# Henningson/Fireflies

Measured on AMD Instinct MI355X. Metric: renders/sec @512x512,64spp vocal-fold (+ pattern-grad-steps/sec in grad_steps_per_sec); HBM GB/s vs peak in roofline, higher is better.
Workload: dtype f32

## Files before the change

fireflies_amd/csrc/ffx_trace.hip:

```cpp
#include <stdlib.h>
#include <string.h>

#include <limits.h>

#include "ffx_common.h"
#include "ffx_band.h"
#include "../../include/ffx_labels.h"

#define TR_BLOCK 256
#define RAY_EPS 8.940696716308594e-05f
#define SHADOW_EPS (10.0f * RAY_EPS)

struct CamK {
  float s2c[16];
  float tw[12];
  float near_clip, far_clip, inv_w, inv_h;
  int W, H;
  int w_uniform;
  float iw_u;
};

struct RfC { float alpha, bias, aL, aL2, k[4]; int rec; };
enum { FFX_PRE_ETA, FFX_PRE_INV_ETA2, FFX_PRE_A2, FFX_PRE_INV_A2, FFX_PRE_METALLIC, FFX_PRE_C_SW, FFX_PRE_C_FD, FFX_PRE_BRDF, FFX_PRE_ROUGH2, FFX_PRE_FLAGS, FFX_PRE_R2,
       FFX_PRE_TINT_TERM, FFX_PRE_FLOATS  };
#define FFX_PRE_ANISO 1u
#define FFX_PRE_TINT 2u
#define FFX_PRE_CLEARCOAT 4u
#define FFX_PRE_FLAT 8u
#define FFX_PRE_SHEEN 16u
// ... 9 lines not shown
  float s_pos[3], s_int[3];
  float cos_cut, cos_beam, cutoff, inv_trans;
  int s_rigid;
  int mat_stride;
  const float *mats;
  int n_base_tex;
  int btw[FFX_MAX_BASE_TEX], bth[FFX_MAX_BASE_TEX];
  const float *btex[FFX_MAX_BASE_TEX];
  const float *slot_uv;
  int mat_inline;
  float mat_h[FFX_MAX_MAT_H];
  int mat_pre_on;
  float mat_pre[8 * FFX_PRE_FLOATS];
  BinsK bins;
  RfC rf;
};
template <typename T>
__device__ __forceinline__ const T &kernarg_first() {
  const __attribute__((address_space(4))) char *p = (const __attribute__((address_space(4))) char *)__builtin_amdgcn_kernarg_segment_ptr();
  asm volatile("" : "+s"(p));
  return *(const T *)p;
}
__device__ __forceinline__ const ShadeK &kernarg_shade() { return kernarg_first<ShadeK>(); }
__device__ __forceinline__ const float *mat_table(const ShadeK &k) { return k.mat_inline ? k.mat_h : k.mats; }

struct Hit { float t; int prim, shape, slot; };

struct RayBox { v3 o, id; };
#define FFX_TIE_WIDEN 1.0000004f
__device__ __forceinline__ float safe_rcp_dir(float d) {
  float a = fabsf(d) < 1e-20f ? copysignf(1e-20f, d) : d;
  return __builtin_amdgcn_rcpf(a);
}
__device__ __forceinline__ RayBox make_raybox(v3 o, v3 d) {
  RayBox r;
  r.o = o;
  r.id = V3(safe_rcp_dir(d.x), safe_rcp_dir(d.y), safe_rcp_dir(d.z));
  return r;
}
__device__ __forceinline__ bool slab(const float lo[3], const float hi[3], const RayBox &rb, float tmin, float tmax, float &tn_out) {
  float ax = (lo[0] - rb.o.x) * rb.id.x, bx = (hi[0] - rb.o.x) * rb.id.x;
  float ay = (lo[1] - rb.o.y) * rb.id.y, by = (hi[1] - rb.o.y) * rb.id.y;
  float az = (lo[2] - rb.o.z) * rb.id.z, bz = (hi[2] - rb.o.z) * rb.id.z;
  float tn = fmaxf(fmaxf(fminf(ax, bx), fminf(ay, by)), fmaxf(fminf(az, bz), tmin));
  float tf = fminf(fminf(fmaxf(ax, bx), fmaxf(ay, by)), fmaxf(az, bz)) * 1.0000004f;
  tf = fminf(tf, tmax);
// ... 103 lines not shown
      if (sp == 0) break;
      --sp;
      cur = stack[sp * stride];
    }
  }
  return h.prim >= 0;
}

__device__ __forceinline__ void sample_jitter(uint32_t seed_key, uint32_t idx, float &jx, float &jy) {
  uint32_t a = hash32((2u * idx) ^ seed_key), b = hash32((2u * idx + 1u) ^ seed_key);
  jx = (float)(a >> 8) * (1.0f / 16777216.0f);
  jy = (float)(b >> 8) * (1.0f / 16777216.0f);
}

#ifdef FFX_K8_NO_BAND
#define FFX_K8_BAND false
#else
#define FFX_K8_BAND true
#endif
#ifdef FFX_K8_NO_OFF32
#define FFX_K8_OFF32 false
#else
#define FFX_K8_OFF32 true
#endif
template <bool BAND = false>
__device__ __forceinline__ void cam_ray(const CamK &k, float sx, float sy, v3 &o, v3 &d, float &near_t, float &far_t) {
  const float *m = k.s2c;
  float qx = fmaf(m[0], sx, fmaf(m[1], sy, m[3]));
  float qy = fmaf(m[4], sx, fmaf(m[5], sy, m[7]));
  float qz = fmaf(m[8], sx, fmaf(m[9], sy, m[11]));
  float iw;
  if (BAND || k.w_uniform) iw = k.iw_u;
  else iw = 1.0f / fmaf(m[12], sx, fmaf(m[13], sy, m[15]));
  v3 np = V3(qx * iw, qy * iw, qz * iw);
  const float il = BAND ? rcp_band(sqrt_band(vdot(np, np))) : 1.0f / sqrtf(vdot(np, np));
  v3 dl = V3(np.x * il, np.y * il, np.z * il);
  d = xf_dir(k.tw, dl);
  o = V3(k.tw[3], k.tw[7], k.tw[11]);
  const float idz = BAND ? rcp_band(dl.z) : 1.0f / dl.z;
  near_t = k.near_clip * idz;
  far_t = k.far_clip * idz;
}

__global__ void __launch_bounds__(TR_BLOCK)
    k_trace_primary(CamK cam, const BvhNode *__restrict__ nodes, const TriRec *__restrict__ recs, int spp, int jitter, uint32_t seed_key, long total,
                    float *__restrict__ t_out, int32_t *__restrict__ shape_out, int32_t *__restrict__ prim_out) {
// ... 1388 lines not shown
    return;
  }
  const float scale = 0.999f * __builtin_amdgcn_rcpf(tmax);
  const RayOct rb = make_rayoct(o, d, scale);
  const uint32_t oct = (__float_as_uint(rb.id.x) >> 31) | ((__float_as_uint(rb.id.y) >> 31) << 1) | ((__float_as_uint(rb.id.z) >> 31) << 2);
  const uint32_t oct0 = (uint32_t)__builtin_amdgcn_readlane((int)oct, __builtin_ctzll(am));
  const bool uniform = (am & __builtin_amdgcn_uicmp(oct, oct0, 33)) == 0ull;
  if (uniform) {
    switch (oct0) {
      case 0: traverse_packet_oct<ANY, 0>(nodes, arecs, rb, scale, d, tmin, tmax, am, h, found); break;
      case 1: traverse_packet_oct<ANY, 1>(nodes, arecs, rb, scale, d, tmin, tmax, am, h, found); break;
      case 2: traverse_packet_oct<ANY, 2>(nodes, arecs, rb, scale, d, tmin, tmax, am, h, found); break;
      case 3: traverse_packet_oct<ANY, 3>(nodes, arecs, rb, scale, d, tmin, tmax, am, h, found); break;
      case 4: traverse_packet_oct<ANY, 4>(nodes, arecs, rb, scale, d, tmin, tmax, am, h, found); break;
      case 5: traverse_packet_oct<ANY, 5>(nodes, arecs, rb, scale, d, tmin, tmax, am, h, found); break;
      case 6: traverse_packet_oct<ANY, 6>(nodes, arecs, rb, scale, d, tmin, tmax, am, h, found); break;
      default: traverse_packet_oct<ANY, 7>(nodes, arecs, rb, scale, d, tmin, tmax, am, h, found); break;
    }
  } else {
    traverse_packet<ANY>(nodes, arecs, o, d, tmin, tmax, active, h, found);
  }
}

template <bool ANY, bool OFF32 = false>
__device__ __forceinline__ void traverse_bins(const char *__restrict__ bbase, const int nx, const int tx0, const int ty0, const int tx1, const int ty1, const float rcx,
                                              const float rcy, const float rhx, const float rhy, const TriApex *__restrict__ recs, const v3 d, const float tmin,
                                              const float tmax, const wmask active, Hit &h, wmask &occluded) {
  h.t = msel(active, tmax, -INFINITY);
  h.prim = -1;
  h.shape = -1;
  h.slot = -1;
  occluded = 0ull;
  const uint32_t lane = threadIdx.x & 63u;
  const uint32_t *starts = reinterpret_cast<const uint32_t *>(bbase + 64);
  const char *ents = bbase + ffx_bin_off_entries();
  const char *rbase = reinterpret_cast<const char *>(recs);
  auto uni = [](float v) { return __int_as_float(__builtin_amdgcn_readfirstlane(__float_as_int(v))); };
  const float rx0 = uni(rcx - rhx), rx1 = uni(rcx + rhx), ry0 = uni(rcy - rhy), ry1 = uni(rcy + rhy);
  FFX_STAT(ANY ? 40 : 32);
  const float tmax_up = tmax * 1.0000038f;
  bool go = true;
  for (int ty = ty0; ty <= ty1 && go; ++ty) {
    for (int tx = tx0; tx <= tx1 && go; ++tx) {
      const uint32_t tile = (uint32_t)(ty * nx + tx);
      const uint32_t beg = starts[tile], end = starts[tile + 1];
      for (uint32_t b0 = beg; b0 < end && go; b0 += 64u) {
        FFX_STAT(ANY ? 41 : 33);
        const uint32_t idx = b0 + lane;
        const uint32_t idc = idx < end ? idx : end - 1u;
        const float4 *e4 = OFF32 ? &at32<float4>(ents, idc << 6) : reinterpret_cast<const float4 *>(ents + ((size_t)idc << 6));
        const float4 A = e4[0], B = e4[1], C = e4[2], D = e4[3];
        wmask m = m_ult(idx, end) & m_le(A.x, rx1) & m_ge(A.z, rx0) & m_le(A.y, ry1) & m_ge(A.w, ry0);
        m &= m_ge(fmaf(B.x, rcx, fmaf(fabsf(B.x), rhx, fmaf(B.y, rcy, fmaf(fabsf(B.y), rhy, B.z)))), 0.f);
        m &= m_ge(fmaf(B.w, rcx, fmaf(fabsf(B.w), rhx, fmaf(C.x, rcy, fmaf(fabsf(C.x), rhy, C.y)))), 0.f);
        m &= m_ge(fmaf(C.z, rcx, fmaf(fabsf(C.z), rhx, fmaf(C.w, rcy, fmaf(fabsf(C.w), rhy, D.x)))), 0.f);
        const int slot_v = __float_as_int(D.y);
        while (m != 0ull) {
          const uint32_t j = (uint32_t)wff1(m);
          asm("s_bitset0_b64 %0, %1" : "+s"(m) : "s"(j));
          FFX_STAT(ANY ? 42 : 34);
          const uint32_t slot = (uint32_t)__builtin_amdgcn_readlane(slot_v, (int)j);
          const uint32_t roff = slot * 48u;
          const v8i r8 = *reinterpret_cast<const v8i *>(rbase + roff);
          const v4i r4 = *reinterpret_cast<const v4i *>(rbase + roff + 32);
          asm volatile("" ::"s"(r8), "s"(r4));
          const int prim = r4.z;
          const v3 Av = V3(__int_as_float(r8.s0), __int_as_float(r8.s1), __int_as_float(r8.s2));
          const v3 Bv = V3(__int_as_float(r8.s3), __int_as_float(r8.s4), __int_as_float(r8.s5));
// ... 16 lines not shown
          const float Vv = vdot(d, Cv);
          const float Vs = msel(neg, -Vv, Vv);
          const wmask p2 = p1 & m_ge(Vs, 0.f) & m_le(Us + Vs, detA);
          if (p2 == 0ull) continue;
          const float t = msel(neg, -T, T) / detA;
          const wmask hitm = p2 & m_gt(t, tmin);
          if (ANY) {
            const wmask occ = hitm & m_lt(t, tmax);
            occluded |= occ;
            msel_into(h.t, occ, -INFINITY);
            if (occ != 0ull && (active & ~occluded) == 0ull) { go = false; m = 0ull; }
          } else {
            const wmask better = hitm & (m_lt(t, h.t) | (m_eq(t, h.t) & m_ult((uint32_t)prim, (uint32_t)h.prim)));
            msel_into(h.t, better, t);
            msel_into(h.prim, better, prim);
            msel_into(h.slot, better, (int)slot);
          }
        }
      }
    }
  }
}

__device__ __forceinline__ bool bins_ready(const BinsK &bk, const int a) {
  if (!bk.g[a].on) return false;
  return reinterpret_cast<const BinHdr *>(bk.base[a])->ok != 0u;
}

template <bool OFF32 = false>
__device__ __forceinline__ bool bins_primary(const BinsK &bk, const int px, const int py, const TriApex *__restrict__ recs, const v3 d, const float tmin, const float tmax,
                                             const wmask active, Hit &h) {
  if (!bins_ready(bk, 0)) return false;
  if (active == 0ull) { h.t = -INFINITY; h.prim = -1; h.shape = -1; h.slot = -1; return true; }
  const float its_x = bk.cam_inv_ts_x, its_y = bk.cam_inv_ts_y;
  const float x0 = (float)px * its_x, y0 = (float)py * its_y;
  const int tx = (int)x0, ty = (int)y0;
  const float hx = 0.5f * its_x - 0.25f * FFX_BIN_PAD, hy = 0.5f * its_y - 0.25f * FFX_BIN_PAD;
  const float cx = x0 + hx, cy = y0 + hy;
  const int stx = __builtin_amdgcn_readfirstlane(tx), sty = __builtin_amdgcn_readfirstlane(ty);
  const float scx = __int_as_float(__builtin_amdgcn_readfirstlane(__float_as_int(cx))), scy = __int_as_float(__builtin_amdgcn_readfirstlane(__float_as_int(cy)));
  const float shx = __int_as_float(__builtin_amdgcn_readfirstlane(__float_as_int(hx))), shy = __int_as_float(__builtin_amdgcn_readfirstlane(__float_as_int(hy)));
  if (stx >= bk.g[0].nx || sty >= bk.g[0].ny) return false;
  wmask occ;
  traverse_bins<false, OFF32>(bk.base[0], bk.g[0].nx, stx, sty, stx, sty, scx, scy, shx, shy, recs, d, tmin, tmax, active, h, occ);
  return true;
}

__device__ __forceinline__ bool bins_block(const BinsK &bk, const int bx0, const int by0, const int bw, const int bh, const TriApex *__restrict__ recs, const v3 d,
                                           const float tmin, const float tmax, const wmask active, Hit &h) {
  if (!bins_ready(bk, 0)) return false;
  if (active == 0ull) { h.t = -INFINITY; h.prim = -1; h.shape = -1; h.slot = -1; return true; }
  const float its_x = bk.cam_inv_ts_x, its_y = bk.cam_inv_ts_y;
  if ((float)bw * its_x > 1.0f || (float)bh * its_y > 1.0f) return false;
  const float x0 = (float)bx0 * its_x, y0 = (float)by0 * its_y;
  const int tx = (int)x0, ty = (int)y0;
  const float hx = 0.5f * (float)bw * its_x - 0.25f * FFX_BIN_PAD, hy = 0.5f * (float)bh * its_y - 0.25f * FFX_BIN_PAD;
  const float cx = x0 + hx, cy = y0 + hy;
  const int stx = __builtin_amdgcn_readfirstlane(tx), sty = __builtin_amdgcn_readfirstlane(ty);
  const float scx = __int_as_float(__builtin_amdgcn_readfirstlane(__float_as_int(cx))), scy = __int_as_float(__builtin_amdgcn_readfirstlane(__float_as_int(cy)));
  const float shx = __int_as_float(__builtin_amdgcn_readfirstlane(__float_as_int(hx))), shy = __int_as_float(__builtin_amdgcn_readfirstlane(__float_as_int(hy)));
  if (stx >= bk.g[0].nx || sty >= bk.g[0].ny) return false;
  wmask occ;
  traverse_bins<false>(bk.base[0], bk.g[0].nx, stx, sty, stx, sty, scx, scy, shx, shy, recs, d, tmin, tmax, active, h, occ);
  return true;
}

__device__ __forceinline__ void wave_reduce_minmax4(uint32_t &mn0, uint32_t &mn1, uint32_t &mx0, uint32_t &mx1) {
#define FFX_R4_STEP(CTRL, MASK)                                                   \
  "v_min_u32_dpp %0, %0, %0 " CTRL " row_mask:" MASK " bank_mask:0xf\n\t"       \
  "v_min_u32_dpp %1, %1, %1 " CTRL " row_mask:" MASK " bank_mask:0xf\n\t"       \
  "v_max_u32_dpp %2, %2, %2 " CTRL " row_mask:" MASK " bank_mask:0xf\n\t"       \
  "v_max_u32_dpp %3, %3, %3 " CTRL " row_mask:" MASK " bank_mask:0xf\n\t"
  asm("s_nop 1\n\t" FFX_R4_STEP("quad_perm:[1,0,3,2]", "0xf") FFX_R4_STEP("quad_perm:[2,3,0,1]", "0xf") FFX_R4_STEP("row_half_mirror", "0xf")
          FFX_R4_STEP("row_mirror", "0xf") FFX_R4_STEP("row_bcast:15", "0xa") FFX_R4_STEP("row_bcast:31", "0xc")
      : "+v"(mn0), "+v"(mn1), "+v"(mx0), "+v"(mx1));
#undef FFX_R4_STEP
  mn0 = (uint32_t)__builtin_amdgcn_readlane((int)mn0, 63);
  mn1 = (uint32_t)__builtin_amdgcn_readlane((int)mn1, 63);
  mx0 = (uint32_t)__builtin_amdgcn_readlane((int)mx0, 63);
  mx1 = (uint32_t)__builtin_amdgcn_readlane((int)mx1, 63);
}

template <bool OFF32 = false>
__device__ __forceinline__ bool bins_shadow(const BinsK &bk, const int a, const TriApex *__restrict__ recs, const v3 sdir, const wmask active, wmask &occluded) {
  if (!bins_ready(bk, a)) return false;
  const float *M = bk.g[a].M;
  const float Z = fmaf(M[6], sdir.x, fmaf(M[7], sdir.y, M[8] * sdir.z));
  const float iz = __builtin_amdgcn_rcpf(Z);
  const float fx = fmaf(M[0], sdir.x, fmaf(M[1], sdir.y, M[2] * sdir.z)) * iz, fy = fmaf(M[3], sdir.x, fmaf(M[4], sdir.y, M[5] * sdir.z)) * iz;
  const float gx = (float)bk.g[a].nx, gy = (float)bk.g[a].ny;
  const wmask inside = m_gt(Z, 0.f) & m_ult(__float_as_uint(fx), __float_as_uint(gx)) & m_ult(__float_as_uint(fy), __float_as_uint(gy));
  if ((active & ~inside) != 0ull) return false;
  if (((bk.env_on >> (a - 1)) & 1) && reinterpret_cast<const BinHdr *>(bk.base[a])->env != 0u) {
    const int nxf = bk.g[a].nx * FFX_ENV_SUB;
    const uint32_t last = (uint32_t)(nxf * bk.g[a].ny * FFX_ENV_SUB) - 1u;
    const uint32_t ci = (uint32_t)((int)(fy * (float)FFX_ENV_SUB) * nxf + (int)(fx * (float)FFX_ENV_SUB));
    const float4 Nc = OFF32 ? at32<float4>(bk.base[a] + bk.env_off, (ci < last ? ci : last) << 4) : reinterpret_cast<const float4 *>(bk.base[a] + bk.env_off)[ci < last ? ci : last];
    const float v = fmaf(Nc.x, sdir.x, fmaf(Nc.y, sdir.y, Nc.z * sdir.z));
    if ((active & ~m_le(v, 1.0f)) == 0ull) { occluded = 0ull; FFX_STAT(a == 1 ? 37 : 47); return true; }
  }
  uint32_t mnx = msel(active, __float_as_uint(fx), 0x7f800000u), mny = msel(active, __float_as_uint(fy), 0x7f800000u);
  uint32_t mxx = msel(active, __float_as_uint(fx), 0u), mxy = msel(active, __float_as_uint(fy), 0u);
  wave_reduce_minmax4(mnx, mny, mxx, mxy);
  const float x0 = __uint_as_float(mnx), y0 = __uint_as_float(mny), x1 = __uint_as_float(mxx), y1 = __uint_as_float(mxy);
  const int tx0 = (int)x0, ty0 = (int)y0, tx1 = (int)x1, ty1 = (int)y1;
  const int stx0 = __builtin_amdgcn_readfirstlane(tx0), sty0 = __builtin_amdgcn_readfirstlane(ty0);
  const int stx1 = __builtin_amdgcn_readfirstlane(tx1), sty1 = __builtin_amdgcn_readfirstlane(ty1);
  if ((stx1 - stx0 + 1) * (sty1 - sty0 + 1) > 4) return false;
  const float cx = 0.5f * (x0 + x1), cy = 0.5f * (y0 + y1), hx = 0.5f * (x1 - x0) + 1e-5f * gx, hy = 0.5f * (y1 - y0) + 1e-5f * gy;
  const float scx = __int_as_float(__builtin_amdgcn_readfirstlane(__float_as_int(cx))), scy = __int_as_float(__builtin_amdgcn_readfirstlane(__float_as_int(cy)));
  const float shx = __int_as_float(__builtin_amdgcn_readfirstlane(__float_as_int(hx))), shy = __int_as_float(__builtin_amdgcn_readfirstlane(__float_as_int(hy)));
  Hit hs;
  traverse_bins<true, OFF32>(bk.base[a], bk.g[a].nx, stx0, sty0, stx1, sty1, scx, scy, shx, shy, recs, sdir, 0.f, 1.0f - SHADOW_EPS, active, hs, occluded);
  return true;
}

struct ShadePre {
  bool ok, need_p, need_s;
  v3 P, ng, Po;
  float pfac, u, v, sfac;
  float pfac_b, sfac_b;
};


template <bool OFF32 = false>
__device__ __forceinline__ bool tex_footprint_lit(const float *__restrict__ tex, int tw, int th, int tc, float u, float v) {
  const float fx = fmaf(u, (float)tw, -0.5f), fy = fmaf(v, (float)th, -0.5f);
  const int ix0 = (int)floorf(fx), iy0 = (int)floorf(fy);
  const int x0 = clampi(ix0, 0, tw - 1), x1 = clampi(ix0 + 1, 0, tw - 1), y0 = clampi(iy0, 0, th - 1), y1 = clampi(iy0 + 1, 0, th - 1);
  float m = 0.f;
  if constexpr (OFF32) {
    const uint32_t r0 = __umul24((uint32_t)y0, (uint32_t)tw), r1 = __umul24((uint32_t)y1, (uint32_t)tw);
    m = fmaxf(m, fmaxf(fmaxf(fabsf(at32<float>(tex, (r0 + (uint32_t)x0) << 2)), fabsf(at32<float>(tex, (r0 + (uint32_t)x1) << 2))),
                       fmaxf(fabsf(at32<float>(tex, (r1 + (uint32_t)x0) << 2)), fabsf(at32<float>(tex, (r1 + (uint32_t)x1) << 2)))));
    return m > 0.f;
  }
  for (int ch = 0; ch < tc; ++ch)
    m = fmaxf(m, fmaxf(fmaxf(fabsf(tex[((size_t)y0 * tw + x0) * tc + ch]), fabsf(tex[((size_t)y0 * tw + x1) * tc + ch])),
                       fmaxf(fabsf(tex[((size_t)y1 * tw + x0) * tc + ch]), fabsf(tex[((size_t)y1 * tw + x1) * tc + ch]))));
  return m > 0.f;
}

template <bool WIDE, int MATM = 0, bool PLAIN = false>
__device__ __forceinline__ void shade_sample_pk(const BvhNode *__restrict__ nodes, const TriRec *__restrict__ recs, const TriApex *__restrict__ arecs,
                                                uint32_t astride, const WideScene &ws, uint2 *__restrict__ stack, const bool &active_, const v3 &o_,
                                                const v3 &d_, const float &nt_, const float &ft_, SampleTerms &st_,
                                                const float4 *__restrict__ nrec, const float4 *__restrict__ gn, const int px, const int py,
                                                const float *__restrict__ tex_probe = nullptr, const int blk_w = 1, const int blk_h = 1) {
  constexpr bool MAT = MATM != 0, TEX = MATM == 2;
  static_assert(!PLAIN || MATM == 1, "the plain-scene instance renders principled rows without textured base colours");
  const bool (&active)[1] = as1(active_);
  const v3 (&o)[1] = as1(o_), (&d)[1] = as1(d_);
  const float (&nt)[1] = as1(nt_), (&ft)[1] = as1(ft_);
  SampleTerms (&st)[1] = as1(st_);
  Hit h[1];
  bool fnd[1];
  FFX_TSTART(tp);
  bool binned = false;
  if (blk_w * blk_h == 1) binned = bins_primary<PLAIN && FFX_K8_OFF32>(kernarg_shade().bins, px, py, arecs, d[0], nt[0], ft[0], wballot(active[0]), h[0]);
  else binned = bins_block(kernarg_shade().bins, px, py, blk_w, blk_h, arecs, d[0], nt[0], ft[0], wballot(active[0]), h[0]);
  if (!binned) {
    FFX_STAT(36);
    traverse_packet_any<false, WIDE>(nodes, arecs, ws, stack, o[0], d[0], nt[0], ft[0], active[0], h[0], fnd[0]);
  }
#ifdef FFX_BINCHECK
  if (binned) {
    Hit h2[1];
    traverse_packet_any<false, WIDE>(nodes, arecs, ws, stack, o[0], d[0], nt[0], ft[0], active[0], h2[0], fnd[0]);
    const bool bad = active[0] && (h2[0].prim != h[0].prim || (h2[0].prim >= 0 && h2[0].t != h[0].t));
    const wmask bm = wballot(bad);
    if (bm != 0ull && (threadIdx.x & 63) == (unsigned)wff1(bm)) {
      atomicAdd(&g_ffx_chk[0], 1ull);
      if (atomicAdd(&g_ffx_chk[1], 1ull) == 0ull) { g_ffx_chk[2] = (unsigned long long)px | ((unsigned long long)py << 16) | ((unsigned long long)(threadIdx.x & 63) << 32); g_ffx_chk[3] = (unsigned long long)(uint32_t)h[0].prim | ((unsigned long long)(uint32_t)h2[0].prim << 32); g_ffx_chk[4] = (unsigned long long)(uint32_t)h[0].slot | ((unsigned long long)(uint32_t)h2[0].slot << 32); g_ffx_chk[5] = (unsigned long long)__float_as_uint(h[0].t) | ((unsigned long long)__float_as_uint(h2[0].t) << 32); }
    }
    h[0] = h2[0];
  }
#endif
  FFX_TSTOP(tp, 22);
  const ShadeK &c = kernarg_shade();
  ShadePre pre[1];
  bool any_p = false, any_s = false;
#pragma unroll
// ... 108 lines not shown
    }
    q.ng = ns;
    if constexpr (!MAT) {
      if (tex_probe && q.need_p) q.need_p = tex_footprint_lit(tex_probe, c.tw, c.th, c.tc, q.u, q.v);
    }
    any_p |= q.need_p;
    any_s |= q.need_s;
  }
  bool occ_p[1], occ_s[1];
  occ_p[0] = occ_s[0] = false;
  FFX_TSTOP(tp, 18);
  const bool walk_p = c.shadows && wballot(any_p) != 0ull, walk_s = c.shadows && wballot(any_s) != 0ull;
  if (walk_p) {
    const v3 ppos = V3(c.p_pos[0], c.p_pos[1], c.p_pos[2]);
    v3 so[1], sdir[1];
    float s0[1], s1[1];
    bool act[1];
    Hit hs[1];
#pragma unroll
    for (int r = 0; r < 1; ++r) { so[r] = ppos; sdir[r] = vsub(pre[r].Po, ppos); s0[r] = 0.f; s1[r] = 1.0f - SHADOW_EPS; act[r] = pre[r].need_p; }
    const TriApex *arecs_p = reinterpret_cast<const TriApex *>(reinterpret_cast<const char *>(arecs) + astride);
    bool binned_p = false;
    wmask occm;
    binned_p = bins_shadow<PLAIN && FFX_K8_OFF32>(kernarg_shade().bins, 1, arecs_p, sdir[0], wballot(act[0]), occm);
    if (binned_p) occ_p[0] = __builtin_amdgcn_inverse_ballot_w64(occm);
    if (!binned_p) {
      FFX_STAT(44);
      traverse_packet_any<true, WIDE>(nodes, arecs_p, ws, stack, so[0], sdir[0], s0[0], s1[0], act[0], hs[0], occ_p[0]);
    }
#ifdef FFX_BINCHECK
    if (binned_p) {
      bool occ2[1];
      traverse_packet_any<true, WIDE>(nodes, arecs_p, ws, stack, so[0], sdir[0], s0[0], s1[0], act[0], hs[0], occ2[0]);
      const wmask bm = wballot(act[0] && occ2[0] != occ_p[0]);
      if (bm != 0ull && (threadIdx.x & 63) == (unsigned)wff1(bm)) {
        atomicAdd(&g_ffx_chk[8], 1ull);
        if (atomicAdd(&g_ffx_chk[9], 1ull) == 0ull) { g_ffx_chk[10] = (unsigned long long)px | ((unsigned long long)py << 16) | ((unsigned long long)(threadIdx.x & 63) << 32) | ((unsigned long long)occ2[0] << 40); g_ffx_chk[11] = (unsigned long long)(uint32_t)hs[0].slot; }
      }
      occ_p[0] = occ2[0];
    }
#endif
  }
  FFX_TSTOP(tp, 19);
  if (walk_s) {
    const v3 spos = V3(c.s_pos[0], c.s_pos[1], c.s_pos[2]);
    v3 so[1], sdir[1];
    float s0[1], s1[1];
    bool act[1];
    Hit hs[1];
#pragma unroll
    for (int r = 0; r < 1; ++r) { so[r] = spos; sdir[r] = vsub(pre[r].Po, spos); s0[r] = 0.f; s1[r] = 1.0f - SHADOW_EPS; act[r] = pre[r].need_s; }
    const TriApex *arecs_s = reinterpret_cast<const TriApex *>(reinterpret_cast<const char *>(arecs) + 2u * astride);
    bool binned_s = false;
    wmask occm;
    binned_s = bins_shadow<PLAIN && FFX_K8_OFF32>(kernarg_shade().bins, 2, arecs_s, sdir[0], wballot(act[0]), occm);
    if (binned_s) occ_s[0] = __builtin_amdgcn_inverse_ballot_w64(occm);
    if (!binned_s) {
      FFX_STAT(45);
      traverse_packet_any<true, WIDE>(nodes, arecs_s, ws, stack, so[0], sdir[0], s0[0], s1[0], act[0], hs[0], occ_s[0]);
    }
#ifdef FFX_BINCHECK
    if (binned_s) {
      bool occ2[1];
      traverse_packet_any<true, WIDE>(nodes, arecs_s, ws, stack, so[0], sdir[0], s0[0], s1[0], act[0], hs[0], occ2[0]);
      const wmask bm = wballot(act[0] && occ2[0] != occ_s[0]);
      if (bm != 0ull && (threadIdx.x & 63) == (unsigned)wff1(bm)) {
        atomicAdd(&g_ffx_chk[16], 1ull);
        if (atomicAdd(&g_ffx_chk[17], 1ull) == 0ull) { g_ffx_chk[18] = (unsigned long long)px | ((unsigned long long)py << 16) | ((unsigned long long)(threadIdx.x & 63) << 32) | ((unsigned long long)occ2[0] << 40); g_ffx_chk[19] = (unsigned long long)(uint32_t)hs[0].slot; }
      }
      occ_s[0] = occ2[0];
    }
#endif
  }
  FFX_TSTOP(tp, 20);
  const ShadeK &c2 = kernarg_shade();
#pragma unroll
  for (int r = 0; r < 1; ++r) {
    ShadePre &q = pre[r];
// ... 338 lines not shown
    float gx[5], gy[5];
    rf_weights(rf, jx, gx);
    rf_weights(rf, jy, gy);
    q[0] = q[1] = q[2] = 0.f;
#pragma unroll
    for (int n = 0; n < 25; ++n) {
      const float w = gx[n % 5] * gy[n / 5];
      q[0] = __builtin_fmaf(w, __uint_as_float((uint32_t)__builtin_amdgcn_readlane((int)__float_as_uint(g[0]), n)), q[0]);
      q[1] = __builtin_fmaf(w, __uint_as_float((uint32_t)__builtin_amdgcn_readlane((int)__float_as_uint(g[1]), n)), q[1]);
      q[2] = __builtin_fmaf(w, __uint_as_float((uint32_t)__builtin_amdgcn_readlane((int)__float_as_uint(g[2]), n)), q[2]);
    }
  }
}

#ifndef FFX_PK_MAT_WAVES
#define FFX_PK_MAT_WAVES 7
#endif
template <int R, bool WIDE, int MATM, bool ADJ = false, bool RF = false, bool RFC = false, bool PLAIN = false, bool CACHE = false>
__global__ void __launch_bounds__(PK_BLOCK) __attribute__((amdgpu_waves_per_eu(MATM ? FFX_PK_MAT_WAVES : FFX_PK1_WAVES, MATM ? FFX_PK_MAT_WAVES : FFX_PK1_WAVES)))
    k_render_fwd_pk(ShadeK c, const BvhNode *__restrict__ nodes, const TriRec *__restrict__ recs, const TriApex *__restrict__ arecs, uint32_t astride,
                    WideScene ws, const float *__restrict__ albedo, const float *__restrict__ tex, int spp, uint32_t seed_key, int tiles_x, int n_tiles, int remap,
                    int fp16, void *__restrict__ img, char *__restrict__ cache, int ppw, float inv_spp_arg, uint32_t cache_foot_off, uint32_t cache_arena_off,
                    uint32_t cache_foot_b_off, const float4 *__restrict__ nrec, const float4 *__restrict__ gn, uint32_t cap_stray,
                    const float *__restrict__ adj_gimg, float *__restrict__ adj_gtex, float *__restrict__ adj_dot) {
  constexpr bool MAT = MATM != 0, TEX = MATM == 2;
  constexpr int MS = MAT ? FFX_MAT_STRIDE : 3;
  constexpr bool CACHE_ARM = !ADJ && !RF && (!PLAIN || CACHE), FOLD_CT = RF ? ADJ : (ADJ || CACHE);
  const bool has_cache = PLAIN ? CACHE : cache != nullptr;
  const bool fold = (RF || PLAIN) ? FOLD_CT : (ADJ || has_cache);
  constexpr int WSTACK_N = WIDE ? FFX_WSTACK : 1, RF_N = (FFX_RF_FLOATS * 4 + 7) / 8;
  __shared__ __attribute__((aligned(16))) uint2 s_wstack[RF ? (WSTACK_N > RF_N ? WSTACK_N : RF_N) : WSTACK_N];
  __shared__ float s_foot[32];
  __shared__ float s_foot_b[MAT ? 32 : 1];
  static_assert(R == 1, "one ray per lane: the adjoint cache is written one pixel at a time");
  static_assert(!RFC || (RF && !ADJ), "RFC: the filtered forward that writes the per-sample adjoint records");
  static_assert(!PLAIN || (MATM == 1 && !RF && !RFC), "PLAIN: principled rows, box film");
  static_assert(!CACHE || (PLAIN && !ADJ), "CACHE: the plain-scene forward that writes the adjoint cache");
  FFX_TINIT();
  FFX_TSTART(twave);
  FFX_TSTART(tpro);
  __shared__ float s_acc[R][RF ? 4 : 3][PK_BLOCK];
  const int wv = __builtin_amdgcn_readfirstlane(xcd_remap(blockIdx.x, gridDim.x, remap) * (blockDim.x >> 6) + (threadIdx.x >> 6));
  const int wpt_log2 = ppw == 1 ? 2 : (ppw == 2 ? 1 : 0);
  const int tile = wv >> wpt_log2, sub0 = (wv & ((1 << wpt_log2) - 1)) * ppw;
  const int lane = threadIdx.x & 63;
  const int W = c.cam.W, H = c.cam.H;
  const int passes = PLAIN ? 1 : (spp + 63) >> 6;
  const float inv_spp_u = inv_spp_arg;
  if constexpr (CACHE_ARM) {
    if (has_cache && wv == 0 && lane == 0) reinterpret_cast<CacheHdr *>(cache)->cap_stray = cap_stray;
  }
  if constexpr (RFC) {
    if (wv == 0 && lane == 0) reinterpret_cast<CacheHdr *>(adj_gtex)->cap_stray = cap_stray;
  }
  FFX_TSTOP(tpro, 25);
  for (int sub = sub0; sub < sub0 + ppw; ++sub) {
    int px[R], py[R];
    packet_pixels<R>(tile, tiles_x, sub, px, py);
    bool live[R], any_live = false;
    uint32_t pix[R];
#pragma unroll
    for (int r = 0; r < R; ++r) {
      live[r] = tile < n_tiles && px[r] < W && py[r] < H;
      any_live |= live[r];
      pix[r] = (uint32_t)py[r] * (uint32_t)W + (uint32_t)px[r];
    }
    if (wballot(any_live) == 0ull) continue;
    int fox = -1, foy = -1, fshape = -1;
    float fin0 = 0.f, fin1 = 0.f, fin2 = 0.f;
    float rfacc[4] = {0.f, 0.f, 0.f, 0.f};
    uint32_t rfc_mask = 0u;
    uint32_t rfc_first = 0u;
    int rfc_first_pass = -1;
    bool rfc_drop = false;
    for (int pass = 0; pass < passes; ++pass) {
      const int s = pass * 64 + lane;
      bool active[R];
      v3 o[R], d[R];
      float nt[R], ft[R];
      FFX_TSTART(tk);
      const CamK &cam = kernarg_shade().cam;
#pragma unroll
      for (int r = 0; r < R; ++r) {
        active[r] = live[r] && s < spp;
        uint32_t idx = pix[r] * (uint32_t)spp + (uint32_t)s;
        float jx, jy;
        sample_jitter(seed_key, idx, jx, jy);
        cam_ray<PLAIN && FFX_K8_BAND>(cam, ((float)px[r] + jx) * cam.inv_w, ((float)py[r] + jy) * cam.inv_h, o[r], d[r], nt[r], ft[r]);
      }
      FFX_TSTOP(tk, 16);
      SampleTerms st[R];
      shade_sample_pk<WIDE, MATM, PLAIN>(nodes, recs, arecs, astride, ws, s_wstack, active[0], o[0], d[0], nt[0], ft[0], st[0], nrec, gn, px[0], py[0], ((fold || RFC) && !(fp16 & 2)) ? nullptr : tex);
      FFX_TSTOP(tk, 17);
      if constexpr (RFC) {
        const bool lit = active[0] && st[0].hit && st[0].has_proj;
        if (wballot(lit) != 0ull && !rfc_drop) {
          char *rfc = reinterpret_cast<char *>(adj_gtex);
          if (rfc_first_pass < 0) {
            const uint32_t want = (uint32_t)(passes - pass);
            if (cap_stray >= (uint32_t)W * (uint32_t)H * (uint32_t)passes) {
              rfc_first = pix[0] * (uint32_t)passes + (uint32_t)pass;
              rfc_first_pass = pass;
            } else {
              const uint32_t sub = ((uint32_t)px[0] + 3u * (uint32_t)py[0]) & 7u, sub_cap = cap_stray >> 3;
              uint32_t b0 = 0u;
              if (lane == 0) b0 = atomicAdd(&reinterpret_cast<CacheHdr *>(rfc)->pad[1 + sub], want);
              b0 = (uint32_t)__builtin_amdgcn_readfirstlane((int)b0);
              if (b0 + want > sub_cap) {
                rfc_drop = true;
                if (lane == 0) atomicAdd(&reinterpret_cast<CacheHdr *>(rfc)->dropped, 1u);
              } else {
                rfc_first = sub * sub_cap + b0;
                rfc_first_pass = pass;
              }
            }
// ... 2371 lines not shown
  };
  if (rf) by_mat(std::true_type());
  else by_mat(std::false_type());
}
template <class F> static void dispatch_rf_dir_amb(bool rf, bool dir, bool amb, F &&f) {
  dispatch_rf_mat(rf, dir, [&](auto r, auto d) {
    if (amb) f(r, d, std::true_type());
    else f(r, d, std::false_type());
  });
}
int ffx_blob_flat(const void *bvh);
static bool plain_scene(const RenderSetup &r, const ffx_scene_desc *sd, const void *bvh, const ffx_bvh_info *info, int fp16) {
  if (!k8_plain_enabled() || r.matm != 1 || !r.c.mat_inline || !r.c.mat_pre_on || (fp16 & FFX_RENDER_FP16) || r.spp > 64) return false;
  if ((r.c.spot_on && !r.c.s_rigid) || (r.c.proj_on && r.c.tc != 1)) return false;
  if (FFX_K8_BAND && !ffx_cam_in_band(r.c.cam.s2c, r.c.cam.w_uniform, r.c.cam.iw_u)) return false;
  if (FFX_K8_OFF32 && (info->total_bytes >= (1ull << 32) || (r.c.proj_on && (r.c.tw >= (1 << 24) || r.c.th >= (1 << 24) || 4ull * (uint64_t)r.c.tw * (uint64_t)r.c.th >= (1ull << 32))))) return false;
  for (int k = 0; k < sd->n_shapes; ++k) {
    uint32_t flags;
    memcpy(&flags, &r.c.mat_pre[k * FFX_PRE_FLOATS + FFX_PRE_FLAGS], 4);
    if (flags != 0u || r.c.mat_h[k * FFX_MAT_STRIDE + FFX_MAT_MODEL] == 0.f) return false;
  }
  return ffx_blob_flat(bvh) == 1;
}
extern "C" { unsigned long long ffx_k8_instance_launches[2] = {0ull, 0ull}; }
struct FwdPkArgs { int fp16; void *img; char *cache; uint32_t off[3], cap_stray; const float *adj_gimg; float *adj_gtex, *adj_dot; bool plain = false; };
template <int ADJ, bool RF = false, bool RFC = false>
static void launch_fwd_pk(bool wide, const RenderSetup &r, const Packets &p, const float *tex, const FwdPkArgs &a, hipStream_t s) {
  dispatch_wm(wide, r.matm, [&](auto w, auto m) {
    auto launch = [&](auto adj) {
      constexpr bool WIDE = decltype(w)::value, A = decltype(adj)::value;
      constexpr int MATM = decltype(m)::value;
      auto go = [&](auto plain, auto with_cache) {
        constexpr bool PLAIN = decltype(plain)::value, CACHE = decltype(with_cache)::value;
        __atomic_fetch_add(&ffx_k8_instance_launches[PLAIN ? 0 : 1], 1ull, __ATOMIC_RELAXED);
        hipLaunchKernelGGL((k_render_fwd_pk<1, WIDE, MATM, A, RF, RFC, PLAIN, CACHE>), dim3(p.pgrid), dim3(64), 0, s, r.c, r.b.nodes, r.b.recs, p.arecs, p.astride, p.ws,
                           r.c.mats, tex, r.spp, r.seed_key, p.ptx, p.pn, xcd_mode(r.n_pix), a.fp16, a.img, a.cache, p.ppw, 1.0f / (float)r.spp, a.off[0],
                           a.off[1], a.off[2], r.b.nrec, r.b.gn, a.cap_stray, a.adj_gimg, a.adj_gtex, a.adj_dot);
      };
      if constexpr ((WIDE || !RF) && (MATM < 2 || (!A && !RFC))) {
        if constexpr (ADJ == 2 && MATM == 1) {
          if (a.plain) {
            if constexpr (!A) {
              if (a.cache) { go(std::true_type(), std::true_type()); return; }
            }
            go(std::true_type(), std::false_type());
            return;
          }
        }
        go(std::false_type(), std::false_type());
      }
    };
    if constexpr (ADJ != 2) launch(std::bool_constant<ADJ == 1>());
    else if (a.adj_gtex) launch(std::true_type());
    else launch(std::false_type());
  });
}
template <bool RF = false>
static void launch_fwd_blk(bool wide, const RenderSetup &r, const Packets &p, const PixBlocks &pb, const float *tex, int fp16, void *img, hipStream_t s) {
  dispatch_wm(wide, r.matm, [&](auto w, auto m) {
    if constexpr (decltype(w)::value || !RF)
// ... 142 lines not shown
      if (sd->proj.enabled && (sd->proj.tex_w > 4094 || sd->proj.tex_h > 4094 || sd->n_shapes > 255)) FFX_FAIL(FFX_ERR_UNSUPPORTED, "render_fwd_cache_filtered: texture larger than 4094^2 or more than 255 shapes");
      if (spp > 1024) FFX_FAIL(FFX_ERR_UNSUPPORTED, "render_fwd_cache_filtered: more than 1024 samples per pixel (16 passes)");
      const size_t n_pix = (size_t)r.n_pix;
      const uint32_t recs_off = (uint32_t)(rfc_off_recs(n_pix) >> 7), facb_off = (uint32_t)(rfc_off_facb(n_pix, (size_t)spp, rfc_all(sd)) >> 7);
      launch_fwd_pk<0, true, true>(true, r, p, tex, {img_fp16, img, (char *)rf_scratch, {recs_off, arena_off, facb_off}, cap_stray, nullptr, (float *)rf_cache, nullptr}, st);
      FFX_CHECK_LAUNCH("render_fwd_cache_filtered");
      return rf_develop(r, img_fp16, img, rf_scratch, st, "render_fwd_cache_filtered/gather", (float *)((char *)rf_cache + rfc_off_wsum(n_pix)));
    }
    if (rf_scratch && spp <= 32 && lowspp_blocks()) {
      launch_fwd_blk<true>(true, r, p, pixel_blocks(r.c.cam, spp, 8, 3), tex, img_fp16 & 1, rf_scratch, st);
      FFX_CHECK_LAUNCH("render_fwd_filtered (pixel blocks)");
      return rf_develop(r, img_fp16, img, rf_scratch, st, "render_fwd_filtered/gather");
    }
    if (rf_scratch) {
      launch_fwd_pk<0, true>(true, r, p, tex, {img_fp16 & 1, img, (char *)rf_scratch, {foot_off, arena_off, foot_b_off}, cap_stray, adj_gimg, adj_gtex, adj_dot}, st);
      FFX_CHECK_LAUNCH("render_fwd_filtered");
      return rf_develop(r, img_fp16, img, rf_scratch, st, "render_fwd_filtered/gather");
    }
    if (!cache && !adj_gtex && spp <= 32 && lowspp_blocks()) {
      launch_fwd_blk(use_wide(info), r, p, pixel_blocks(r.c.cam, spp, 1, spp == 1 ? 4 : 3), tex, img_fp16, img, st);
      FFX_CHECK_LAUNCH("render_fwd (pixel blocks)");
      return FFX_OK;
    }
    launch_fwd_pk<2>(use_wide(info), r, p, tex, {img_fp16, img, (char *)cache, {foot_off, arena_off, foot_b_off}, cap_stray, adj_gimg, adj_gtex, adj_dot, plain_scene(r, sd, bvh, info, img_fp16)}, st);
    FFX_CHECK_LAUNCH("render_fwd");
    return FFX_OK;
  }
  int tiles_x = ffx_cdiv(r.c.cam.W, 8), tiles_y = ffx_cdiv(r.c.cam.H, 8);
  int n_tiles = tiles_x * tiles_y;
  int grid = ((n_tiles + 7) / 8) * 8;
  hipLaunchKernelGGL(k_render_fwd, dim3(grid), dim3(TR_BLOCK), stack_bytes(info), st, r.c, r.b.nodes, r.b.recs, r.b.nrec, shape_albedo, tex, spp,
                     r.seed_key, tiles_x, n_tiles, xcd_mode(), img_fp16, img);
  FFX_CHECK_LAUNCH("render_fwd");
  return FFX_OK;
}

#define FFX_NO_APPEARANCE(flags_, what_)                                                                                                                  \
  do {                                                                                                                                                    \
    if ((flags_) & FFX_RENDER_GRAD_APPEARANCE) FFX_FAIL(FFX_ERR_UNSUPPORTED, "%s: FFX_RENDER_GRAD_APPEARANCE is served by ffx_render_bwd[_filtered] only", what_); \
    if ((flags_) & FFX_RENDER_GRAD_MATERIAL) FFX_FAIL(FFX_ERR_UNSUPPORTED, "%s: FFX_RENDER_GRAD_MATERIAL is served by ffx_render_bwd[_filtered] only", what_);     \
    if ((flags_) & FFX_RENDER_GRAD_PRB) FFX_FAIL(FFX_ERR_UNSUPPORTED, "%s: FFX_RENDER_GRAD_PRB is served by ffx_render_bwd[_filtered] only", what_);               \
  } while (0)
#define FFX_NO_TANGENT(flags_, what_) \
  do { if ((flags_) & FFX_RENDER_TANGENT) FFX_FAIL(FFX_ERR_UNSUPPORTED, "%s: FFX_RENDER_TANGENT is served by ffx_render_fwd[_filtered] only", what_); } while (0)
static int render_jvp(const void *bvh, const ffx_bvh_info *info, const ffx_scene_desc *sd, const float *shape_albedo, const float *tex, int spp, uint32_t seed,
                      int img_fp16, void *img, ffx_stream s, void *rf_scratch) {
  const char *what = rf_scratch ? "render_fwd_filtered" : "render_fwd";
// ... 678 lines not shown
```

Baseline: 3590.

## Precompute per-pixel bin rectangle table and use scalar constant loads in plain K8 path

Adds a host-built, device-cached table of per-pixel bin centers, rect bounds and tile indices, read through constant address-space loads in the primary binned traversal of the plain, non-cache K8 instance. It also makes the packet's pixel coordinates wave-uniform, passes float grid extents via kernarg for shadow bins, and reads bin starts and headers as scalar loads. The aim is to replace per-lane float math, readfirstlane and vector loads with uniform scalar loads. The cost is an extra kernel argument, a global table cache guarded by a mutex with a fixed slot count, and a one-time synchronous upload.

```diff
diff --git a/fireflies_amd/csrc/ffx_rect.h b/fireflies_amd/csrc/ffx_rect.h
--- /dev/null
+++ b/fireflies_amd/csrc/ffx_rect.h
@@ -0,0 +1,37 @@
+#ifndef FFX_RECT_H
+#define FFX_RECT_H
+#include <cstdint>
+#include <cstring>
+#include <vector>
+
+#define FFX_RECT_BIN_PAD 0.00390625f
+#define FFX_RECT_MAX_SIDE 4096
+
+struct FfxRectEntry { float c, r0, r1; int32_t t; };
+static_assert(sizeof(FfxRectEntry) == 16, "a rectangle entry is one 16-byte scalar load");
+
+static inline float ffx_rect_half(float its) { return 0.5f * its - 0.25f * FFX_RECT_BIN_PAD; }
+
+static inline FfxRectEntry ffx_rect_entry(int p, float its) {
+  const float x0 = (float)p * its;
+  const float h = ffx_rect_half(its);
+  const float c = x0 + h;
+  FfxRectEntry e;
+  e.c = c;
+  e.r0 = c - h;
+  e.r1 = c + h;
+  e.t = (int)x0;
+  return e;
+}
+
+static inline bool ffx_rect_fill(int W, int H, float its_x, float its_y, std::vector<FfxRectEntry> &tab, float &hx, float &hy) {
+  if (W < 1 || H < 1 || W > FFX_RECT_MAX_SIDE || H > FFX_RECT_MAX_SIDE) return false;
+  if (!(its_x > 0.f) || !(its_y > 0.f) || its_x > 1.f || its_y > 1.f) return false;
+  tab.resize((size_t)W + (size_t)H);
+  for (int px = 0; px < W; ++px) tab[(size_t)px] = ffx_rect_entry(px, its_x);
+  for (int py = 0; py < H; ++py) tab[(size_t)W + (size_t)py] = ffx_rect_entry(py, its_y);
+  hx = ffx_rect_half(its_x);
+  hy = ffx_rect_half(its_y);
+  return true;
+}
+#endif
diff --git a/fireflies_amd/csrc/ffx_trace.hip b/fireflies_amd/csrc/ffx_trace.hip
--- a/fireflies_amd/csrc/ffx_trace.hip
+++ b/fireflies_amd/csrc/ffx_trace.hip
@@ -2,9 +2,11 @@
 #include <string.h>
 
 #include <limits.h>
+#include <mutex>
 
 #include "ffx_common.h"
 #include "ffx_band.h"
+#include "ffx_rect.h"
 #include "../../include/ffx_labels.h"
 
 #define TR_BLOCK 256
@@ -60,6 +62,8 @@
   return *(const T *)p;
 }
 __device__ __forceinline__ const ShadeK &kernarg_shade() { return kernarg_first<ShadeK>(); }
+struct RectK { const void *tab; float hx, hy; uint32_t row0, pad; float gxf[FFX_N_APEX], gyf[FFX_N_APEX]; };
+__device__ __forceinline__ const RectK &kernarg_rect();
 __device__ __forceinline__ const float *mat_table(const ShadeK &k) { return k.mat_inline ? k.mat_h : k.mats; }
 
 struct Hit { float t; int prim, shape, slot; };
@@ -209,6 +213,26 @@
 #define FFX_K8_OFF32 false
 #else
 #define FFX_K8_OFF32 true
+#endif
+#ifdef FFX_K8_NO_RECTTAB
+#define FFX_K8_RECTTAB false
+#else
+#define FFX_K8_RECTTAB true
+#endif
+#ifdef FFX_K8_NO_RECT_UNI
+#define FFX_K8_RECT_UNI false
+#else
+#define FFX_K8_RECT_UNI true
+#endif
+#ifdef FFX_K8_NO_RECT_GF
+#define FFX_K8_RECT_GF false
+#else
+#define FFX_K8_RECT_GF true
+#endif
+#ifdef FFX_K8_NO_RECT_SL
+#define FFX_K8_RECT_SL false
+#else
+#define FFX_K8_RECT_SL true
 #endif
 template <bool BAND = false>
 __device__ __forceinline__ void cam_ray(const CamK &k, float sx, float sy, v3 &o, v3 &d, float &near_t, float &far_t) {
@@ -1643,10 +1667,12 @@
   }
 }
 
-template <bool ANY, bool OFF32 = false>
+#define FFX_CONST_AS __attribute__((address_space(4)))
+template <bool ANY, bool OFF32 = false, bool BOX = false, bool SL = false>
 __device__ __forceinline__ void traverse_bins(const char *__restrict__ bbase, const int nx, const int tx0, const int ty0, const int tx1, const int ty1, const float rcx,
                                               const float rcy, const float rhx, const float rhy, const TriApex *__restrict__ recs, const v3 d, const float tmin,
-                                              const float tmax, const wmask active, Hit &h, wmask &occluded) {
+                                              const float tmax, const wmask active, Hit &h, wmask &occluded, const float bx0 = 0.f, const float bx1 = 0.f,
+                                              const float by0 = 0.f, const float by1 = 0.f) {
   h.t = msel(active, tmax, -INFINITY);
   h.prim = -1;
   h.shape = -1;
@@ -1657,14 +1683,20 @@
   const char *ents = bbase + ffx_bin_off_entries();
   const char *rbase = reinterpret_cast<const char *>(recs);
   auto uni = [](float v) { return __int_as_float(__builtin_amdgcn_readfirstlane(__float_as_int(v))); };
-  const float rx0 = uni(rcx - rhx), rx1 = uni(rcx + rhx), ry0 = uni(rcy - rhy), ry1 = uni(rcy + rhy);
+  const float rx0 = BOX ? bx0 : uni(rcx - rhx), rx1 = BOX ? bx1 : uni(rcx + rhx), ry0 = BOX ? by0 : uni(rcy - rhy), ry1 = BOX ? by1 : uni(rcy + rhy);
   FFX_STAT(ANY ? 40 : 32);
   const float tmax_up = tmax * 1.0000038f;
   bool go = true;
   for (int ty = ty0; ty <= ty1 && go; ++ty) {
     for (int tx = tx0; tx <= tx1 && go; ++tx) {
       const uint32_t tile = (uint32_t)(ty * nx + tx);
-      const uint32_t beg = starts[tile], end = starts[tile + 1];
+      uint32_t beg, end;
+      if constexpr (SL) {
+        const FFX_CONST_AS uint32_t *sc = (const FFX_CONST_AS uint32_t *)(uintptr_t)starts;
+        beg = sc[tile]; end = sc[tile + 1];
+      } else {
+        beg = starts[tile]; end = starts[tile + 1];
+      }
       for (uint32_t b0 = beg; b0 < end && go; b0 += 64u) {
         FFX_STAT(ANY ? 41 : 33);
         const uint32_t idx = b0 + lane;
@@ -1727,16 +1759,30 @@
   }
 }
 
+template <bool SL = false>
 __device__ __forceinline__ bool bins_ready(const BinsK &bk, const int a) {
   if (!bk.g[a].on) return false;
-  return reinterpret_cast<const BinHdr *>(bk.base[a])->ok != 0u;
-}
-
-template <bool OFF32 = false>
+  if constexpr (SL) return ((const FFX_CONST_AS BinHdr *)(uintptr_t)bk.base[a])->ok != 0u;
+  else return reinterpret_cast<const BinHdr *>(bk.base[a])->ok != 0u;
+}
+
+typedef float v4f __attribute__((ext_vector_type(4)));
+template <bool OFF32 = false, bool RECT = false, bool SL = false>
 __device__ __forceinline__ bool bins_primary(const BinsK &bk, const int px, const int py, const TriApex *__restrict__ recs, const v3 d, const float tmin, const float tmax,
                                              const wmask active, Hit &h) {
-  if (!bins_ready(bk, 0)) return false;
+  if (!bins_ready<SL>(bk, 0)) return false;
   if (active == 0ull) { h.t = -INFINITY; h.prim = -1; h.shape = -1; h.slot = -1; return true; }
+  if constexpr (RECT) {
+    typedef const __attribute__((address_space(4))) v4f *ctab;
+    const RectK &rk = kernarg_rect();
+    const ctab tab = (ctab)(uintptr_t)rk.tab;
+    const v4f ex = tab[(uint32_t)px], ey = tab[rk.row0 + (uint32_t)py];
+    const int stx = __float_as_int(ex.w), sty = __float_as_int(ey.w);
+    if (stx >= bk.g[0].nx || sty >= bk.g[0].ny) return false;
+    wmask occ;
+    traverse_bins<false, OFF32, true, SL>(bk.base[0], bk.g[0].nx, stx, sty, stx, sty, ex.x, ey.x, rk.hx, rk.hy, recs, d, tmin, tmax, active, h, occ, ex.y, ex.z, ey.y, ey.z);
+    return true;
+  }
   const float its_x = bk.cam_inv_ts_x, its_y = bk.cam_inv_ts_y;
   const float x0 = (float)px * its_x, y0 = (float)py * its_y;
   const int tx = (int)x0, ty = (int)y0;
@@ -1747,7 +1793,7 @@
   const float shx = __int_as_float(__builtin_amdgcn_readfirstlane(__float_as_int(hx))), shy = __int_as_float(__builtin_amdgcn_readfirstlane(__float_as_int(hy)));
   if (stx >= bk.g[0].nx || sty >= bk.g[0].ny) return false;
   wmask occ;
-  traverse_bins<false, OFF32>(bk.base[0], bk.g[0].nx, stx, sty, stx, sty, scx, scy, shx, shy, recs, d, tmin, tmax, active, h, occ);
+  traverse_bins<false, OFF32, false, SL>(bk.base[0], bk.g[0].nx, stx, sty, stx, sty, scx, scy, shx, shy, recs, d, tmin, tmax, active, h, occ);
   return true;
 }
 
@@ -1786,17 +1832,23 @@
   mx1 = (uint32_t)__builtin_amdgcn_readlane((int)mx1, 63);
 }
 
-template <bool OFF32 = false>
+template <bool OFF32 = false, bool GF = false, bool SL = false>
 __device__ __forceinline__ bool bins_shadow(const BinsK &bk, const int a, const TriApex *__restrict__ recs, const v3 sdir, const wmask active, wmask &occluded) {
-  if (!bins_ready(bk, a)) return false;
+  if (!bins_ready<SL>(bk, a)) return false;
   const float *M = bk.g[a].M;
   const float Z = fmaf(M[6], sdir.x, fmaf(M[7], sdir.y, M[8] * sdir.z));
   const float iz = __builtin_amdgcn_rcpf(Z);
   const float fx = fmaf(M[0], sdir.x, fmaf(M[1], sdir.y, M[2] * sdir.z)) * iz, fy = fmaf(M[3], sdir.x, fmaf(M[4], sdir.y, M[5] * sdir.z)) * iz;
-  const float gx = (float)bk.g[a].nx, gy = (float)bk.g[a].ny;
+  float gx, gy;
+  if constexpr (GF) { gx = kernarg_rect().gxf[a]; gy = kernarg_rect().gyf[a]; }
+  else { gx = (float)bk.g[a].nx; gy = (float)bk.g[a].ny; }
   const wmask inside = m_gt(Z, 0.f) & m_ult(__float_as_uint(fx), __float_as_uint(gx)) & m_ult(__float_as_uint(fy), __float_as_uint(gy));
   if ((active & ~inside) != 0ull) return false;
-  if (((bk.env_on >> (a - 1)) & 1) && reinterpret_cast<const BinHdr *>(bk.base[a])->env != 0u) {
+  auto env_built = [&]() {
+    if constexpr (SL) return ((const FFX_CONST_AS BinHdr *)(uintptr_t)bk.base[a])->env != 0u;
+    else return reinterpret_cast<const BinHdr *>(bk.base[a])->env != 0u;
+  };
+  if (((bk.env_on >> (a - 1)) & 1) && env_built()) {
     const int nxf = bk.g[a].nx * FFX_ENV_SUB;
     const uint32_t last = (uint32_t)(nxf * bk.g[a].ny * FFX_ENV_SUB) - 1u;
     const uint32_t ci = (uint32_t)((int)(fy * (float)FFX_ENV_SUB) * nxf + (int)(fx * (float)FFX_ENV_SUB));
@@ -1816,7 +1868,7 @@
   const float scx = __int_as_float(__builtin_amdgcn_readfirstlane(__float_as_int(cx))), scy = __int_as_float(__builtin_amdgcn_readfirstlane(__float_as_int(cy)));
   const float shx = __int_as_float(__builtin_amdgcn_readfirstlane(__float_as_int(hx))), shy = __int_as_float(__builtin_amdgcn_readfirstlane(__float_as_int(hy)));
   Hit hs;
-  traverse_bins<true, OFF32>(bk.base[a], bk.g[a].nx, stx0, sty0, stx1, sty1, scx, scy, shx, shy, recs, sdir, 0.f, 1.0f - SHADOW_EPS, active, hs, occluded);
+  traverse_bins<true, OFF32, false, SL>(bk.base[a], bk.g[a].nx, stx0, sty0, stx1, sty1, scx, scy, shx, shy, recs, sdir, 0.f, 1.0f - SHADOW_EPS, active, hs, occluded);
   return true;
 }
 
@@ -1846,7 +1898,7 @@
   return m > 0.f;
 }
 
-template <bool WIDE, int MATM = 0, bool PLAIN = false>
+template <bool WIDE, int MATM = 0, bool PLAIN = false, bool RECT = false>
 __device__ __forceinline__ void shade_sample_pk(const BvhNode *__restrict__ nodes, const TriRec *__restrict__ recs, const TriApex *__restrict__ arecs,
                                                 uint32_t astride, const WideScene &ws, uint2 *__restrict__ stack, const bool &active_, const v3 &o_,
                                                 const v3 &d_, const float &nt_, const float &ft_, SampleTerms &st_,
@@ -1862,7 +1914,7 @@
   bool fnd[1];
   FFX_TSTART(tp);
   bool binned = false;
-  if (blk_w * blk_h == 1) binned = bins_primary<PLAIN && FFX_K8_OFF32>(kernarg_shade().bins, px, py, arecs, d[0], nt[0], ft[0], wballot(active[0]), h[0]);
+  if (blk_w * blk_h == 1) binned = bins_primary<PLAIN && FFX_K8_OFF32, RECT, RECT && FFX_K8_RECT_SL>(kernarg_shade().bins, px, py, arecs, d[0], nt[0], ft[0], wballot(active[0]), h[0]);
   else binned = bins_block(kernarg_shade().bins, px, py, blk_w, blk_h, arecs, d[0], nt[0], ft[0], wballot(active[0]), h[0]);
   if (!binned) {
     FFX_STAT(36);
@@ -2017,7 +2069,7 @@
     const TriApex *arecs_p = reinterpret_cast<const TriApex *>(reinterpret_cast<const char *>(arecs) + astride);
     bool binned_p = false;
     wmask occm;
-    binned_p = bins_shadow<PLAIN && FFX_K8_OFF32>(kernarg_shade().bins, 1, arecs_p, sdir[0], wballot(act[0]), occm);
+    binned_p = bins_shadow<PLAIN && FFX_K8_OFF32, RECT && FFX_K8_RECT_GF, RECT && FFX_K8_RECT_SL>(kernarg_shade().bins, 1, arecs_p, sdir[0], wballot(act[0]), occm);
     if (binned_p) occ_p[0] = __builtin_amdgcn_inverse_ballot_w64(occm);
     if (!binned_p) {
       FFX_STAT(44);
@@ -2048,7 +2100,7 @@
     const TriApex *arecs_s = reinterpret_cast<const TriApex *>(reinterpret_cast<const char *>(arecs) + 2u * astride);
     bool binned_s = false;
     wmask occm;
-    binned_s = bins_shadow<PLAIN && FFX_K8_OFF32>(kernarg_shade().bins, 2, arecs_s, sdir[0], wballot(act[0]), occm);
+    binned_s = bins_shadow<PLAIN && FFX_K8_OFF32, RECT && FFX_K8_RECT_GF, RECT && FFX_K8_RECT_SL>(kernarg_shade().bins, 2, arecs_s, sdir[0], wballot(act[0]), occm);
     if (binned_s) occ_s[0] = __builtin_amdgcn_inverse_ballot_w64(occm);
     if (!binned_s) {
       FFX_STAT(45);
@@ -2433,7 +2485,7 @@
                     WideScene ws, const float *__restrict__ albedo, const float *__restrict__ tex, int spp, uint32_t seed_key, int tiles_x, int n_tiles, int remap,
                     int fp16, void *__restrict__ img, char *__restrict__ cache, int ppw, float inv_spp_arg, uint32_t cache_foot_off, uint32_t cache_arena_off,
                     uint32_t cache_foot_b_off, const float4 *__restrict__ nrec, const float4 *__restrict__ gn, uint32_t cap_stray,
-                    const float *__restrict__ adj_gimg, float *__restrict__ adj_gtex, float *__restrict__ adj_dot) {
+                    const float *__restrict__ adj_gimg, float *__restrict__ adj_gtex, float *__restrict__ adj_dot, RectK rk) {
   constexpr bool MAT = MATM != 0, TEX = MATM == 2;
   constexpr int MS = MAT ? FFX_MAT_STRIDE : 3;
   constexpr bool CACHE_ARM = !ADJ && !RF && (!PLAIN || CACHE), FOLD_CT = RF ? ADJ : (ADJ || CACHE);
@@ -2465,9 +2517,13 @@
     if (wv == 0 && lane == 0) reinterpret_cast<CacheHdr *>(adj_gtex)->cap_stray = cap_stray;
   }
   FFX_TSTOP(tpro, 25);
+  constexpr bool RECT_I = PLAIN && !CACHE && FFX_K8_RECTTAB, UNI = RECT_I && FFX_K8_RECT_UNI;
+  int bx0[R], by0[R];
+  if constexpr (UNI) packet_pixels<R>(tile, tiles_x, 0, bx0, by0);
   for (int sub = sub0; sub < sub0 + ppw; ++sub) {
     int px[R], py[R];
-    packet_pixels<R>(tile, tiles_x, sub, px, py);
+    if constexpr (UNI) { px[0] = bx0[0] + (sub & 1); py[0] = by0[0] + (sub >> 1); }
+    else packet_pixels<R>(tile, tiles_x, sub, px, py);
     bool live[R], any_live = false;
     uint32_t pix[R];
 #pragma unroll
@@ -2476,7 +2532,11 @@
       any_live |= live[r];
       pix[r] = (uint32_t)py[r] * (uint32_t)W + (uint32_t)px[r];
     }
-    if (wballot(any_live) == 0ull) continue;
+    if constexpr (UNI) {
+      if (!any_live) continue;
+    } else {
+      if (wballot(any_live) == 0ull) continue;
+    }
     int fox = -1, foy = -1, fshape = -1;
     float fin0 = 0.f, fin1 = 0.f, fin2 = 0.f;
     float rfacc[4] = {0.f, 0.f, 0.f, 0.f};
@@ -2501,7 +2561,7 @@
       }
       FFX_TSTOP(tk, 16);
       SampleTerms st[R];
-      shade_sample_pk<WIDE, MATM, PLAIN>(nodes, recs, arecs, astride, ws, s_wstack, active[0], o[0], d[0], nt[0], ft[0], st[0], nrec, gn, px[0], py[0], ((fold || RFC) && !(fp16 & 2)) ? nullptr : tex);
+      shade_sample_pk<WIDE, MATM, PLAIN, RECT_I>(nodes, recs, arecs, astride, ws, s_wstack, active[0], o[0], d[0], nt[0], ft[0], st[0], nrec, gn, px[0], py[0], ((fold || RFC) && !(fp16 & 2)) ? nullptr : tex);
       FFX_TSTOP(tk, 17);
       if constexpr (RFC) {
         const bool lit = active[0] && st[0].hit && st[0].has_proj;
@@ -4919,8 +4979,66 @@
   }
   return ffx_blob_flat(bvh) == 1;
 }
+static_assert(FFX_RECT_BIN_PAD == FFX_BIN_PAD, "ffx_rect.h restates the bins' pad");
+#define FFX_RECT_KEYS 32
+struct RectTab { int dev, W, H; float its_x, its_y, hx, hy; void *d; };
+static RectTab g_rect_tab[FFX_RECT_KEYS];
+static std::mutex g_rect_mu;
+static bool rect_tables(const ShadeK &c, RectK &rk, hipStream_t s) {
+  const BinsK &bk = c.bins;
+  memset(&rk, 0, sizeof rk);
+  for (int a = 0; a < FFX_N_APEX; ++a) { rk.gxf[a] = (float)bk.g[a].nx; rk.gyf[a] = (float)bk.g[a].ny; }
+  if (!bk.g[0].on) return true;
+  const int W = c.cam.W, H = c.cam.H;
+  int dev = 0;
+  if (hipGetDevice(&dev) != hipSuccess) return false;
+  std::lock_guard<std::mutex> lock(g_rect_mu);
+  RectTab *e = nullptr, *free_slot = nullptr;
+  for (RectTab &t : g_rect_tab) {
+    if (t.d && t.dev == dev && t.W == W && t.H == H && t.its_x == bk.cam_inv_ts_x && t.its_y == bk.cam_inv_ts_y) { e = &t; break; }
+    if (!t.d && !free_slot) free_slot = &t;
+  }
+  if (!e) {
+    if (!free_slot) {
+      static bool told = false;
+      if (!told) fprintf(stderr, "libffx_hip: all %d pixel-rectangle tables are in use; further film sizes render through the generic K8 instance\n", FFX_RECT_KEYS);
+      told = true;
+      return false;
+    }
+    std::vector<FfxRectEntry> tab;
+    float hx, hy;
+    if (!ffx_rect_fill(W, H, bk.cam_inv_ts_x, bk.cam_inv_ts_y, tab, hx, hy)) return false;
+    void *d = nullptr;
+    if (hipMalloc(&d, tab.size() * sizeof(FfxRectEntry)) != hipSuccess) { (void)hipGetLastError(); return false; }
+    if (hipMemcpyAsync(d, tab.data(), tab.size() * sizeof(FfxRectEntry), hipMemcpyHostToDevice, s) != hipSuccess || hipStreamSynchronize(s) != hipSuccess) {
+      (void)hipGetLastError();
+      (void)hipFree(d);
+      return false;
+    }
+    *free_slot = {dev, W, H, bk.cam_inv_ts_x, bk.cam_inv_ts_y, hx, hy, d};
+    e = free_slot;
+  }
+  rk.tab = e->d;
+  rk.hx = e->hx;
+  rk.hy = e->hy;
+  rk.row0 = (uint32_t)W;
+  return true;
+}
 extern "C" { unsigned long long ffx_k8_instance_launches[2] = {0ull, 0ull}; }
-struct FwdPkArgs { int fp16; void *img; char *cache; uint32_t off[3], cap_stray; const float *adj_gimg; float *adj_gtex, *adj_dot; bool plain = false; };
+template <class F> struct KernargLast;
+template <class... A> struct KernargLast<void (*)(A...)> {
+  static constexpr size_t offset() {
+    size_t off = 0, last = 0;
+    ((off = (off + alignof(A) - 1) / alignof(A) * alignof(A), last = off, off += sizeof(A)), ...);
+    return last;
+  }
+};
+__device__ __forceinline__ const RectK &kernarg_rect() {
+  const __attribute__((address_space(4))) char *p = (const __attribute__((address_space(4))) char *)__builtin_amdgcn_kernarg_segment_ptr();
+  asm volatile("" : "+s"(p));
+  return *(const RectK *)(p + KernargLast<decltype(&k_render_fwd_pk<1, true, 1>)>::offset());
+}
+struct FwdPkArgs { int fp16; void *img; char *cache; uint32_t off[3], cap_stray; const float *adj_gimg; float *adj_gtex, *adj_dot; bool plain = false; RectK rk = {}; };
 template <int ADJ, bool RF = false, bool RFC = false>
 static void launch_fwd_pk(bool wide, const RenderSetup &r, const Packets &p, const float *tex, const FwdPkArgs &a, hipStream_t s) {
   dispatch_wm(wide, r.matm, [&](auto w, auto m) {
@@ -4932,7 +5050,7 @@
         __atomic_fetch_add(&ffx_k8_instance_launches[PLAIN ? 0 : 1], 1ull, __ATOMIC_RELAXED);
         hipLaunchKernelGGL((k_render_fwd_pk<1, WIDE, MATM, A, RF, RFC, PLAIN, CACHE>), dim3(p.pgrid), dim3(64), 0, s, r.c, r.b.nodes, r.b.recs, p.arecs, p.astride, p.ws,
                            r.c.mats, tex, r.spp, r.seed_key, p.ptx, p.pn, xcd_mode(r.n_pix), a.fp16, a.img, a.cache, p.ppw, 1.0f / (float)r.spp, a.off[0],
-                           a.off[1], a.off[2], r.b.nrec, r.b.gn, a.cap_stray, a.adj_gimg, a.adj_gtex, a.adj_dot);
+                           a.off[1], a.off[2], r.b.nrec, r.b.gn, a.cap_stray, a.adj_gimg, a.adj_gtex, a.adj_dot, a.rk);
       };
       if constexpr ((WIDE || !RF) && (MATM < 2 || (!A && !RFC))) {
         if constexpr (ADJ == 2 && MATM == 1) {
@@ -5121,7 +5239,10 @@
       FFX_CHECK_LAUNCH("render_fwd (pixel blocks)");
       return FFX_OK;
     }
-    launch_fwd_pk<2>(use_wide(info), r, p, tex, {img_fp16, img, (char *)cache, {foot_off, arena_off, foot_b_off}, cap_stray, adj_gimg, adj_gtex, adj_dot, plain_scene(r, sd, bvh, info, img_fp16)}, st);
+    RectK rk = {};
+    const bool reads_tables = FFX_K8_RECTTAB && (adj_gtex || !cache);
+    const bool plain = plain_scene(r, sd, bvh, info, img_fp16) && (!reads_tables || rect_tables(r.c, rk, st));
+    launch_fwd_pk<2>(use_wide(info), r, p, tex, {img_fp16, img, (char *)cache, {foot_off, arena_off, foot_b_off}, cap_stray, adj_gimg, adj_gtex, adj_dot, plain, rk}, st);
     FFX_CHECK_LAUNCH("render_fwd");
     return FFX_OK;
   }
```

Result: faster. 3745 (median of 6 runs) (+4.3%).
